# Xiaoming-Zhao/PointNav-VO

Hardware: AMD Instinct MI355X
Metric: RGB-D frame-pair VO inferences/s @341x192 (higher is better)
Workload: dtype f32

## Files before the change

### pointnav-vo_amd/csrc/pnvo_api.hip

```cpp
#include <hip/hip_runtime.h>

#include <cmath>
#include <cstdio>
#include <cstdlib>
#include <cstring>
#include <functional>
#include <atomic>
#include <condition_variable>
#include <map>
#include <mutex>
#include <string>
#include <thread>
#include <vector>

#include "pnvo_model.h"

using namespace pnvo;

thread_local std::string g_err;

int pnvo_fail(pnvo_handle h, int code, const std::string &msg) {
  if (h) h->err = msg;
  g_err = msg;
  return code;
}

long long pnvo_device_bytes_live(void) { return g_device_bytes_live.load(); }

namespace {

inline int fail(pnvo_handle h, int code, const std::string &msg) { return pnvo_fail(h, code, msg); }


Layer make_layer(const std::string &name, const std::string &gn, int cin, int cout, int k, int stride, int pad,
                 int hin, int win, int groups) {
  Layer l;
  l.name = name;
  l.gn = gn;
  l.cin = cin;
  l.cinp = rup(cin, 8);
  l.cout = cout;
  l.coutp = rup(cout, 32);
  l.k = l.kw = k;
  l.stride = stride;
  l.pad = pad;
  l.hin = hin;
  l.win = win;
  l.hout = (hin + 2 * pad - k) / stride + 1;
  l.wout = (win + 2 * pad - k) / stride + 1;
  l.groups = groups;
  return l;
}

void build_plan(pnvo_model_s *m) {
  const pnvo_config &c = m->cfg;
  m->C = c.n_rgb + c.n_depth + c.n_dd + c.n_tdv;
  m->CP = rup(m->C, 8);
  m->CPL = rup(m->C, 16);
  m->Hs = halve(c.height);
  m->Ws = halve(c.width);
  m->Hp = halve(m->Hs);
  m->Wp = halve(m->Ws);
  {
    const int n[4] = {c.n_rgb, c.n_depth, c.n_dd, c.n_tdv};
    int prev_off[4], half = 0;
    for (int t = 0; t < 4; ++t) {
      prev_off[t] = half;
      half += n[t] / 2;
    }
    m->stem_ref_of_new.clear();
    m->stem_tensor_of_new.clear();
    m->stem_ch_of_new.clear();
    for (int t = 0; t < 4; ++t)
      for (int ch = 0; ch < n[t]; ++ch) {
        const int hn = n[t] / 2;
        m->stem_ref_of_new.push_back(ch < hn ? prev_off[t] + ch : half + prev_off[t] + (ch - hn));
        m->stem_tensor_of_new.push_back(t);
        m->stem_ch_of_new.push_back(ch);
      }
    while ((int)m->stem_ref_of_new.size() < m->CP) {
      m->stem_ref_of_new.push_back(-1);
      m->stem_tensor_of_new.push_back(-1);
      m->stem_ch_of_new.push_back(0);
    }
  }
  const int g = c.baseplanes / 2;
  const std::string bb = "visual_encoder.backbone.";
  m->convs.clear();
  m->convs.push_back(make_layer(bb + "conv1.0", bb + "conv1.1", m->C, c.baseplanes, 7, 2, 3, c.height, c.width, g));
  int h = m->Hp, w = m->Wp, cin = c.baseplanes;
  const bool bott = c.backbone_depth == 50 || c.backbone_depth == 101;
  const int nblk[4] = {bott ? 3 : 2, bott ? 4 : 2, bott ? (c.backbone_depth == 101 ? 23 : 6) : 2, bott ? 3 : 2};
  const bool resnext = bott && c.resnext != 0, se = bott && c.se != 0;
  const int expansion = resnext ? 2 : 4, cardinality = resnext ? c.baseplanes / 2 : 1;
  m->bottleneck = bott;
  m->grouped_se = resnext || se;
  m->blocks.clear();
  auto push = [&](Layer l) {
    l.block = (int)m->blocks.size();
    m->convs.push_back(std::move(l));
    return (int)m->convs.size() - 1;
  };
  for (int st = 1; st <= 4; ++st) {
    const int planes = (resnext ? 2 * c.baseplanes : c.baseplanes) << (st - 1), cout = bott ? planes * expansion : planes;
    for (int bi = 0; bi < nblk[st - 1]; ++bi) {
      Block b;
      b.stage = st;
      b.index = bi;
      b.tap = "layer" + std::to_string(st) + "." + std::to_string(bi);
      const std::string p = bb + b.tap + ".";
      const int stride = (st > 1 && bi == 0) ? 2 : 1;
      if (bott) {
        Layer b2 = make_layer(p + "convs.3", p + "convs.4", planes, planes, 3, stride, 1, h, w, g);
        b.nconv = 3;
        b.conv[0] = push(make_layer(p + "convs.0", p + "convs.1", cin, planes, 1, 1, 0, h, w, g));
        if (bi == 0) b2.cgroups = cardinality;
        const int h2 = b2.hout, w2 = b2.wout;
        b.conv[1] = push(std::move(b2));
        if (se) b.se_r = cout / 16;
        b.conv[2] = push(make_layer(p + "convs.6", p + "convs.7", planes, cout, 1, 1, 0, h2, w2, g));
      } else {
        Layer c1 = make_layer(p + "convs.0", p + "convs.1", cin, planes, 3, stride, 1, h, w, g);
        b.nconv = 2;
        const int h1 = c1.hout, w1 = c1.wout;
        b.conv[0] = push(std::move(c1));
        b.conv[1] = push(make_layer(p + "convs.3", p + "convs.4", planes, planes, 3, 1, 1, h1, w1, g));
      }
      if (stride != 1 || cin != cout) b.ds = push(make_layer(p + "downsample.0", p + "downsample.1", cin, cout, 1, stride, 0, h, w, g));
      m->blocks.push_back(std::move(b));
      h = m->last(m->blocks.back()).hout;
      w = m->last(m->blocks.back()).wout;
      cin = cout;
    }
  }
  m->fh = h;
  m->fw = w;
  m->comp_c = (int)std::lround((double)c.flat_size / (double)(h * w));
  {
    const double q = (double)c.flat_size / (double)(h * w);
    const double fl = std::floor(q);
    if (q - fl == 0.5) m->comp_c = ((long)fl % 2 == 0) ? (int)fl : (int)fl + 1;
  }
  m->comp_cp = rup(m->comp_c, 32);
  m->comp = (int)m->convs.size();
  m->convs.push_back(make_layer("visual_encoder.compression.0", "visual_encoder.compression.1", cin, m->comp_c, 3, 1, 1,
                                h, w, 1));
  m->fc = make_layer(c.act_embed ? "hidden_generator.1" : "visual_fc.2", "", m->comp_c, c.hidden, 1, 1, 0, h, w, 1);
  m->fc.cinp = m->comp_cp;
  m->fc.k = h;
  m->fc.kw = w;
  m->fc.hout = m->fc.wout = 1;
  m->head = make_layer("output_head.1", "", c.hidden, c.out_dim, 1, 1, 0, 1, 1, 1);
}

struct Toc {
  std::map<std::string, const pnvo_tensor_desc *> by_name;
  const float *blob;
  size_t n;
};

const float *find_tensor(pnvo_handle h, const Toc &t, const std::string &name, std::vector<int64_t> shape, int *rc) {
  auto it = t.by_name.find(name);
  if (it == t.by_name.end()) {
    *rc = fail(h, PNVO_ERR_WEIGHTS, "state_dict is missing tensor '" + name + "'");
    return nullptr;
  }
  const pnvo_tensor_desc *d = it->second;
// ... 684 lines not shown
static int stem_launch_mx(pnvo_handle m, int B, const StemRequest &r, const StemPlan &p, GnGroup &sgg) {
  const Layer &stem = m->convs[0];
  StemMXArgs a;
  std::memset(&a, 0, sizeof(a));
  pnvo_stem_mx_input(m, B, r.src, r.raw, a);
  a.wpk = p.pieces == 2 ? m->mx_wpk2 : m->mx_wpk3;
  a.oscale = m->mx_oscale;
  a.oscale_ptr = m->mx_wpk2_dev ? m->mx_scale2_dev + 1 : nullptr;
  a.bad_input = m->dd_flag_dev;
  const int ntn = stem.cout / 32;
  for (int g = 0; g < ntn; ++g) {
    a.y[g] = r.y;
    a.stats[g] = m->stats;
    a.y_coff[g] = 32 * g;
  }
  a.y_cstride = stem.coutp;
  a.stats_cstride = stem.coutp;
  a.pool = r.pool_keys;
  a.pool_gamma = stem.gamma;
  a.Hp = m->Hp;
  a.Wp = m->Wp;
  if (r.grp != nullptr) {
    if (p.pieces != 2 || r.pool_keys == nullptr) return fail(m, PNVO_ERR_STATE, "grouped forward needs the float16-piece stem with pooled keys");
    a.grp_end0 = sgg.end0 = r.grp->end[0];
    if (r.grp->n > 2) a.grp_end1 = sgg.end1 = r.grp->end[1];
    for (int k = 1; k < r.grp->n; ++k) {
      pnvo_handle hk = r.grp->h[k];
      if (hk->mx_wpk2 == nullptr || hk->mx_wpk2_dev) return fail(m, PNVO_ERR_STATE, "grouped forward: a model has no host-packed float16 stem operand");
      a.wpk_g[k - 1] = hk->mx_wpk2;
      a.oscale_g[k - 1] = hk->mx_oscale;
      a.pool_gamma_g[k - 1] = sgg.gamma[k - 1] = hk->convs[0].gamma;
      sgg.beta[k - 1] = hk->convs[0].beta;
    }
  }
  a.dbg = m->opt.stem_dbg >= 16 ? m->opt.stem_dbg - 16 : 0;
  if (m->opt.stem_dbg == 9 || m->opt.stem_dbg >= 16) {
    if (!m->mx_prof) {
      HIPCHK(m, m->mx_prof.alloc(256));
      HIPCHK(m, hipMemset(m->mx_prof, 0, 2048));
    }
    a.prof = m->mx_prof;
  }
  if (p.standin) return pnvo_stem_standin(m, B, r, p.slots, nullptr);
  Timed t = stem_timed(m, B, r, false);
  return pnvo_launch_stem_mx(m, a, p.pieces, ntn, false, r.grp, r.s);
}

static int stem_launch_dd(pnvo_handle m, int B, const StemRequest &r, const StemPlan &p) {
  const pnvo_config &c = m->cfg;
  if (p.standin) return pnvo_stem_standin(m, B, r, p.slots, nullptr);
  const int nsrc[4] = {c.n_rgb, c.n_depth, c.n_dd, c.n_tdv};
  StemDDArgs a;
  std::memset(&a, 0, sizeof(a));
  for (int j = 0; j < 3; ++j)
    for (int q = 0; q < 2; ++q) {
      const int d = 4 * j + 2 * q;
      const int tn = m->dd_dense_tensor[d];
      a.pieces[j][0][q].base = tn >= 0 ? r.src[tn] : nullptr;
      a.pieces[j][0][q].nch = tn >= 0 ? nsrc[tn] : 0;
      a.pieces[j][0][q].choff = tn >= 0 ? m->dd_dense_ch[d] : 0;
    }
  a.sc = m->dd_sc;
  a.sh = m->dd_sh;
  a.wpk = m->dd_wpk;
  a.table = m->dd_table;
  a.dd = r.src[2];
  a.zero_page = m->zero_page;
  a.bad_onehot = m->dd_flag_dev;
  a.y = r.y;
  a.stats = m->stats;
  a.B = B;
  a.H = c.height;
  a.W = c.width;
  a.Ho = m->Hs;
  a.Wo = m->Ws;
  a.bins = m->dd_bins;
  a.slots = p.slots;
  a.dbg = m->opt.stem_dbg;
  if (a.dbg == 9) {
    if (!m->dd_prof) {
      HIPCHK(m, m->dd_prof.alloc(8));
      HIPCHK(m, hipMemset(m->dd_prof, 0, 64));
    }
    a.prof = m->dd_prof;
  }
  Timed t = stem_timed(m, B, r, false);
  HIPCHK(m, launch_stem_dd(a, r.s));
  return PNVO_OK;
}

int pnvo_run_stem(pnvo_handle m, int B, const StemRequest &r) {
  const Layer &stem = m->convs[0];
  const StemPlan p = pnvo_stem_plan(m, r.train_fwd, r.raw);
  int rc = PNVO_OK;
  if (r.pool_keys != nullptr && !p.pools()) return fail(m, PNVO_ERR_STATE, "pooled stem output asked of a stem kernel without it");
  GnGroup sgg{0x7fffffff, 0x7fffffff, {nullptr, nullptr}, {nullptr, nullptr}};
  switch (p.kernel) {
    case StemPlan::MX: rc = stem_launch_mx(m, B, r, p, sgg); break;
    case StemPlan::DD: rc = stem_launch_dd(m, B, r, p); break;
    case StemPlan::LDS: {
      StemArgs a;
      stem_lds_args(m, B, r, p.slots, a);
      a.dbg = m->opt.stem_dbg;
      a.lds_pad = m->opt.stem_dbg_pad;
      Timed t = stem_timed(m, B, r, false);
      HIPCHK(m, launch_stem_lds(a, stem.coutp, r.s));
      break;
    }
    case StemPlan::GENERIC:
      return pnvo_run_conv(m, stem, B, {.in_scale = m->stem_sc, .in_shift = m->stem_sh, .y = r.y, .y_cstride = stem.coutp, .ss = r.ss,
                                        .mu = r.mu, .rstd = r.rstd, .src = r.src, .grp = r.grp, .s = r.s});
  }
  if (rc != PNVO_OK) return rc;
  if (p.kernel != StemPlan::LDS) {
    if (p.repairs && (rc = pnvo_stem_standin(m, B, r, p.slots, m->dd_flag_dev)) != PNVO_OK) return rc;
    if ((rc = pnvo_mark_stem(m, r.s, p)) != PNVO_OK) return rc;
  }
  if (r.slots_out != nullptr) *r.slots_out = p.slots;
  if (!r.skip_finalize) {
    Timed t(m, r.s, "gn_finalize", 0.0, 0.0);
    HIPCHK(m, launch_gn_finalize(m->stats, B, p.slots, stem.coutp, stem.cout, stem.groups, (long)m->Hs * m->Ws, 1, stem.gamma, stem.beta,
                                 1e-5f, r.ss[0], r.ss[1], r.s, p.slots, r.mu, r.rstd, r.grp ? &sgg : nullptr));
  }
  return PNVO_OK;
}

int pnvo_ensure_workspace(pnvo_handle m, int B) { return ensure_workspace(m, B); }

namespace {
struct OptChoice {
  const char *word;
  int value;
};
struct OptDef {
  const char *key, *env;
  int PnvoOptions::*field;
  bool numeric;
  OptChoice choices[7];
};
const OptDef kOptions[] = {
    {"stem", "PNVO_STEM", &PnvoOptions::stem, false, {{"auto", 0}, {"mx", 1}, {"dd", 2}, {"dense", 3}, {nullptr, 0}}},
    {"conv", "PNVO_CONV", &PnvoOptions::conv, false, {{"auto", 0}, {"x3", 1}, {"fp32", 2}, {"generic", 3}, {nullptr, 0}}},
    {"pieces", "PNVO_PIECES", &PnvoOptions::pieces, false, {{"2", 2}, {"3", 3}, {nullptr, 0}}},
    {"stem_form", "PNVO_STEM_FORM", &PnvoOptions::stem_form, false, {{"auto", 0}, {"tiles", 2}, {"resident", 3}, {"fast", 4}, {nullptr, 0}}},
    {"train_pieces", "PNVO_TRAIN_PIECES", &PnvoOptions::train_pieces, false, {{"2", 2}, {"3", 3}, {nullptr, 0}}},
    {"x3_persist", "PNVO_X3_PERSIST", &PnvoOptions::x3_persist, false, {{"on", 1}, {"off", 0}, {nullptr, 0}}},
    {"x3_rows", "PNVO_X3_ROWS", &PnvoOptions::x3_rows, false, {{"on", 1}, {"off", 0}, {nullptr, 0}}},
    {"x3_strip", "PNVO_X3_STRIP", &PnvoOptions::x3_strip, false, {{"on", 1}, {"off", 0}, {nullptr, 0}}},
    {"x3_fine", "PNVO_X3_FINE", &PnvoOptions::x3_fine, false, {{"on", 1}, {"off", 0}, {nullptr, 0}}},
    {"x3_w8", "PNVO_X3_W8", &PnvoOptions::x3_w8, false, {{"on", 1}, {"off", 0}, {nullptr, 0}}},
    {"x3_m16", "PNVO_X3_M16", &PnvoOptions::x3_m16, false, {{"on", 1}, {"off", 0}, {nullptr, 0}}},
    {"x3_ksplit", "PNVO_X3_KSPLIT", &PnvoOptions::x3_ksplit, false, {{"on", 1}, {"off", 0}, {nullptr, 0}}},
    {"fc_rows", "PNVO_FC_ROWS", &PnvoOptions::fc_rows, true, {{nullptr, 0}}},
    {"head_fuse", "PNVO_HEAD_FUSE", &PnvoOptions::head_fuse, false, {{"on", 1}, {"off", 0}, {nullptr, 0}}},
    {"ds_fuse", "PNVO_DS_FUSE", &PnvoOptions::ds_fuse, false, {{"on", 1}, {"off", 0}, {nullptr, 0}}},
    {"gn_fuse", "PNVO_GN_FUSE", &PnvoOptions::gn_fuse, false, {{"on", 1}, {"off", 0}, {nullptr, 0}}},
    {"x3_s2", nullptr, &PnvoOptions::x3_s2, false, {{"on", 1}, {"off", 0}, {nullptr, 0}}},
    {"tail", "PNVO_TAIL", &PnvoOptions::tail, false, {{"fused", 1}, {"separate", 0}, {nullptr, 0}}},
    {"pool", "PNVO_POOL", &PnvoOptions::pool, false, {{"fused", 1}, {"separate", 0}, {nullptr, 0}}},
    {"graph", "PNVO_GRAPH", &PnvoOptions::graph, true, {{nullptr, 0}}},
    {"stem_dbg", nullptr, &PnvoOptions::stem_dbg, true, {{nullptr, 0}}},
    {"stem_dbg_pad", nullptr, &PnvoOptions::stem_dbg_pad, true, {{nullptr, 0}}},
    {"wgrad_stem", "PNVO_WGRAD_STEM", &PnvoOptions::wgrad_stem, false, {{"mx", 0}, {"fp32", 1}, {nullptr, 0}}},
    {"wgrad3", "PNVO_WGRAD3", &PnvoOptions::wgrad3, false, {{"x3", 1}, {"fp32", 0}, {nullptr, 0}}},
    {"pool_bwd", "PNVO_POOL_BWD", &PnvoOptions::pool_bwd, false, {{"fused", 1}, {"separate", 0}, {nullptr, 0}}},
    {"dgrad", "PNVO_DGRAD", &PnvoOptions::dgrad, false, {{"phase", 1}, {"masked", 0}, {nullptr, 0}}},
    {"bf16_fuse", nullptr, &PnvoOptions::bf16_fuse, false, {{"on", 1}, {"off", 0}, {nullptr, 0}}},
    {"input_fallback", "PNVO_INPUT_FALLBACK", &PnvoOptions::input_fallback, false, {{"on", 1}, {"off", 0}, {nullptr, 0}}},
    {"small_net", "PNVO_SMALL_NET", &PnvoOptions::small_net, false, {{"on", 1}, {"off", 0}, {nullptr, 0}}},
    {"small_max", "PNVO_SMALL_MAX", &PnvoOptions::small_max, true, {{nullptr, 0}}},
    {"small_coop", "PNVO_SMALL_COOP", &PnvoOptions::small_coop, true, {{nullptr, 0}}},
    {"small_prof", "PNVO_SMALL_PROF", &PnvoOptions::small_prof, true, {{nullptr, 0}}},
};

const OptDef *find_option(const char *key) {
  for (const OptDef &d : kOptions)
    if (std::strcmp(d.key, key) == 0) return &d;
  return nullptr;
}

bool parse_option(const OptDef &d, const char *word, int *out) {
  if (d.numeric) {
    char *end = nullptr;
    const long v = std::strtol(word, &end, 10);
    if (end == word || *end != 0) return false;
    *out = (int)v;
    return true;
  }
  for (const OptChoice *c = d.choices; c->word != nullptr; ++c)
    if (std::strcmp(c->word, word) == 0) {
      *out = c->value;
      return true;
    }
  return false;
}

void env_defaults(pnvo_model_s *m) {
  for (const OptDef &d : kOptions) {
    const char *e = d.env ? std::getenv(d.env) : nullptr;
    int v;
    if (e && parse_option(d, e, &v)) m->opt.*(d.field) = v;
  }
  if (std::getenv("PNVO_X3_S2_OFF")) m->opt.x3_s2 = 0;
  if (std::getenv("PNVO_BF16_NOFUSE")) m->opt.bf16_fuse = 0;
  if (const char *e = std::getenv("PNVO_STEM_DBG")) std::sscanf(e, "%d,%d", &m->opt.stem_dbg, &m->opt.stem_dbg_pad);
}
}


int pnvo_input_fallback(pnvo_handle m, hipStream_t s, bool *rerun) {
  *rerun = false;
  if (!m->stem_ev_pending) return PNVO_OK;
  m->stem_ev_pending = false;
  HIPCHK(m, hipEventSynchronize(m->stem_ev));
  if (!m->dd_flag || *(volatile int *)m->dd_flag == 0) return PNVO_OK;
  *(volatile int *)m->dd_flag = 0;
  HIPCHK(m, hipMemsetAsync(m->dd_flag_dev, 0, sizeof(int), s));
  m->dense_sticky = true;
  m->fallback_count += 1;
  pnvo_drop_graphs(m);
  m->note = "note: observation values outside the fused stems' contract (fractional rgb or depth codes that are not one-hot) — "
           "the forward was re-run on the dense fp32 stem and this handle stays on it";
  *rerun = true;
  return PNVO_OK;
}

namespace {
int forward_dispatch(pnvo_handle m, int B, const FwdRequest &r);
int forward_body(pnvo_handle m, int B, const FwdRequest &r);
}


extern "C" {

#include "src_hash.h"
const char *pnvo_version(void) { return "pnvo 0.3 (gfx950: fp32 + f16/bf16 MFMA) src:" PNVO_SRC_HASH; }

const char *pnvo_last_error(pnvo_handle h) { return h ? h->err.c_str() : g_err.c_str(); }

const char *pnvo_last_note(pnvo_handle h) {
  if (h && h->loaded && h->opt.input_fallback && pnvo_stem_plan(h, false, {}).lds_serves) (void)pnvo_check_inputs(h);
  return h ? h->note.c_str() : "";
}

int pnvo_create(const pnvo_config *cfg, int device, pnvo_handle *out) {
  if (!cfg || !out) return fail(nullptr, PNVO_ERR_ARG, "null argument");
  const int C = cfg->n_rgb + cfg->n_depth + cfg->n_dd + cfg->n_tdv;
  if (C <= 0) return fail(nullptr, PNVO_ERR_ARG, "visual odometry must not be blind (no input modality)");
  if (C > 64 || (cfg->n_rgb % 2) || (cfg->n_depth % 2) || (cfg->n_dd % 2) || (cfg->n_tdv % 2))
    return fail(nullptr, PNVO_ERR_ARG, "unsupported input channel configuration");
  if (cfg->width < 32 || cfg->height < 32) return fail(nullptr, PNVO_ERR_ARG, "observation_size must be >= 32x32");
  if (cfg->baseplanes < 32 || cfg->baseplanes % 32 || cfg->hidden % 8 || cfg->hidden <= 0 || cfg->out_dim <= 0)
    return fail(nullptr, PNVO_ERR_ARG, "unsupported baseplanes / hidden_size / output_dim");
  if ((cfg->resnext != 0 && cfg->resnext != 1) || (cfg->se != 0 && cfg->se != 1) ||
      ((cfg->resnext || cfg->se) && cfg->backbone_depth != 50 && cfg->backbone_depth != 101))
    return fail(nullptr, PNVO_ERR_ARG, "unsupported backbone: resnext / se are 0 or 1 and need backbone_depth 50 or 101");
  hipError_t e = hipSetDevice(device);
  if (e != hipSuccess) return fail(nullptr, PNVO_ERR_HIP, std::string("hipSetDevice: ") + hipGetErrorString(e));
  hipDeviceProp_t prop;
  e = hipGetDeviceProperties(&prop, device);
  if (e != hipSuccess) return fail(nullptr, PNVO_ERR_HIP, std::string("hipGetDeviceProperties: ") + hipGetErrorString(e));
  if (std::string(prop.gcnArchName).rfind("gfx950", 0) != 0)
    return fail(nullptr, PNVO_ERR_ARG, std::string("libpnvo is built for gfx950 only, device is ") + prop.gcnArchName);
  pnvo_model_s *m = new pnvo_model_s();
  static std::atomic<unsigned long long> next_uid{1};
  m->uid = next_uid.fetch_add(1);
  m->cfg = *cfg;
  m->device = device;
  m->num_cus = prop.multiProcessorCount;
  if (m->cfg.flat_size <= 0) m->cfg.flat_size = 2048;
  if (m->cfg.n_acts <= 0) m->cfg.n_acts = 4;
  env_defaults(m);
  build_plan(m);
  *out = m;
  return PNVO_OK;
}

int pnvo_load_weights(pnvo_handle h, const float *blob, size_t n_floats, const pnvo_tensor_desc *toc, int ntoc) {
  if (!h || !blob || !toc) return fail(h, PNVO_ERR_ARG, "null argument");
  HIPCHK(h, hipSetDevice(h->device));
  pnvo_drop_graphs(h);
  Toc t;
  t.blob = blob;
  t.n = n_floats;
  for (int k = 0; k < ntoc; ++k) t.by_name[toc[k].name] = &toc[k];
  int rc = PNVO_OK;
  const pnvo_config &c = h->cfg;
  h->mean.assign(h->C, 0.f);
  h->stdev.assign(h->C, 1.f);
  if (c.normalize) {
    const std::string pre = "visual_encoder.running_mean_and_var.";
    const float *mu = find_tensor(h, t, pre + "_mean", {1, h->C, 1, 1}, &rc);
    if (!mu) return rc;
    const float *var = find_tensor(h, t, pre + "_var", {1, h->C, 1, 1}, &rc);
    if (!var) return rc;
    for (int k = 0; k < h->C; ++k) {
      h->mean[k] = mu[k];
      h->stdev[k] = std::sqrt(std::fmax(var[k], 1e-2f));
    }
  }
  for (Layer &l : h->convs)
    if ((rc = load_conv(h, t, l, true)) != PNVO_OK) return rc;
  for (Block &b : h->blocks) {
    if (b.se_r == 0) continue;
    const std::string pre = "visual_encoder.backbone." + b.tap + ".se.excite.";
    const int C = h->last(b).cout, R = b.se_r;
    if (!se_gate_supported(C, R)) return fail(h, PNVO_ERR_ARG, "SE branch of " + b.tap + ": unsupported width " + std::to_string(C));
// ... 496 lines not shown
      if (b.se_r > 0) {
        if (b3.cout != b3.coutp) return fail(m, PNVO_ERR_STATE, "SE block " + b.tap + " on a channel-padded map");
        Timed t(m, s, "se_gate:" + b.tap, 2.0 * B * (2.0 * b.se_r + (double)Pb) * b3.cout, 4.0 * B * Pb * b3.cout);
        HIPCHK(m, launch_se_gate({.x = m->rawB, .scale = m->ssA[0], .shift = m->ssA[1], .w1 = b.se_w1, .b1 = b.se_b1, .w2 = b.se_w2,
                                  .b2 = b.se_b2, .out_scale = m->ssE[0], .out_shift = m->ssE[1], .B = B, .P = (int)Pb, .C = b3.cout,
                                  .R = b.se_r}, s));
        ss3 = m->ssE;
      }
      if (ds) {
        const Layer &cd = m->convs[b.ds];
        if ((rc = pnvo_run_conv(m, cd, B, {.x = cur, .y = m->rawD, .y_cstride = cd.coutp, .ss = m->ssD, .grp = grp, .s = s})) != PNVO_OK)
          return rc;
        Timed t(m, s, "residual", 0.0, 12.0 * B * Pb * b3.coutp);
        HIPCHK(m, launch_residual(m->rawB, ss3[0], ss3[1], m->rawD, m->ssD[0], m->ssD[1], B, Pb, b3.coutp, nxt, s));
      } else {
        Timed t(m, s, "residual", 0.0, 12.0 * B * Pb * b3.coutp);
        HIPCHK(m, launch_residual(m->rawB, ss3[0], ss3[1], cur, nullptr, nullptr, B, Pb, b3.coutp, nxt, s));
      }
      std::swap(cur, nxt);
      if ((rc = maybe_tap(m, b.tap.c_str(), cur, (size_t)B * Pb * b3.coutp, s)) != PNVO_OK) return rc;
      continue;
    }
    const Layer &c1 = m->convs[b.conv[0]];
    const Layer &c2 = m->convs[b.conv[1]];
    const bool ds_ride = ds && !have_keys && pnvo_conv_takes_ds(m, c1, m->convs[b.ds], B);
    const DsRide ride{ds_ride ? &m->convs[b.ds] : nullptr, m->rawD, m->ssD, nullptr, nullptr};
    if (have_keys) {
      BlockTail ktail{nullptr, nullptr, nullptr, cur};
      if ((rc = pnvo_run_conv(m, c1, B, {.x = nxt, .in_scale = m->ssA[0], .in_shift = m->ssA[1], .y = m->rawA, .y_cstride = c1.coutp,
                                         .ss = m->ssA, .tail = &ktail, .grp = grp, .s = s})) != PNVO_OK)
        return rc;
      have_keys = false;
    } else if (have_tail) {
      if (ds_ride) tail.out = nullptr;
      if ((rc = pnvo_run_conv(m, c1, B, {.x = m->rawB, .in_scale = m->ssB[0], .in_shift = m->ssB[1], .y = m->rawA, .y_cstride = c1.coutp,
                                         .ss = m->ssA, .tail = &tail, .ride = ds_ride ? &ride : nullptr, .grp = grp, .s = s})) != PNVO_OK)
        return rc;
      std::swap(cur, nxt);
      have_tail = false;
    } else if ((rc = pnvo_run_conv(m, c1, B, {.x = cur, .y = m->rawA, .y_cstride = c1.coutp, .ss = m->ssA, .ride = ds_ride ? &ride : nullptr,
                                              .grp = grp, .s = s})) != PNVO_OK) {
      return rc;
    }
    const long P = (long)c2.hout * c2.wout;
    const bool c2_small_generic = !layer_on_lds(m, c2, nullptr) && !pnvo_conv_on_x3(m, c2, B) && (size_t)B * P * c2.cinp * 4 <= ((size_t)48 << 20);
    if (c2_small_generic) {
      float *napp = ds_ride ? nxt : m->rawD;
      {
        Timed t(m, s, "gn_relu_apply", 0.0, 8.0 * B * P * c2.cinp);
        HIPCHK(m, launch_apply_ss_relu(m->rawA, m->ssA[0], m->ssA[1], B, P, c2.cinp, napp, s));
      }
      if ((rc = pnvo_run_conv(m, c2, B, {.x = napp, .y = m->rawB, .y_cstride = c2.coutp, .ss = m->ssB, .grp = grp, .s = s})) != PNVO_OK)
        return rc;
    } else if ((rc = pnvo_run_conv(m, c2, B, {.x = m->rawA, .in_scale = m->ssA[0], .in_shift = m->ssA[1], .y = m->rawB, .y_cstride = c2.coutp,
                                              .ss = m->ssB, .grp = grp, .s = s})) != PNVO_OK) {
      return rc;
    }
    if (ds) {
      const Layer &cd = m->convs[b.ds];
      if (!ds_ride &&
          (rc = pnvo_run_conv(m, cd, B, {.x = cur, .y = m->rawD, .y_cstride = cd.coutp, .ss = m->ssD, .grp = grp, .s = s})) != PNVO_OK)
        return rc;
    }
    if (pnvo_conv_takes_tail(m, m->convs[m->next_conv_after(bk)], B)) {
      tail.res = ds ? m->rawD : cur;
      tail.res_scale = ds ? m->ssD[0] : nullptr;
      tail.res_shift = ds ? m->ssD[1] : nullptr;
      tail.out = nxt;
      have_tail = true;
      continue;
    }
    {
      Timed t(m, s, "residual", 0.0, 12.0 * B * P * c2.coutp);
      HIPCHK(m, launch_residual(m->rawB, m->ssB[0], m->ssB[1], ds ? m->rawD : cur, ds ? m->ssD[0] : nullptr, ds ? m->ssD[1] : nullptr, B,
                                P, c2.coutp, nxt, s));
    }
    std::swap(cur, nxt);
    if ((rc = maybe_tap(m, b.tap.c_str(), cur, (size_t)B * P * c2.coutp, s)) != PNVO_OK) return rc;
  }

  const Layer &comp = m->convs[m->comp];
  if (have_tail) {
    tail.out = nullptr;
    if ((rc = pnvo_run_conv(m, comp, B, {.x = m->rawB, .in_scale = m->ssB[0], .in_shift = m->ssB[1], .y = m->comp_raw, .y_cstride = comp.coutp,
                                         .ss = m->ssC, .tail = &tail, .grp = grp, .s = s})) != PNVO_OK)
      return rc;
    have_tail = false;
  } else if ((rc = pnvo_run_conv(m, comp, B, {.x = cur, .y = m->comp_raw, .y_cstride = comp.coutp, .ss = m->ssC, .grp = grp, .s = s})) != PNVO_OK) {
    return rc;
  }
  if (m->tap_dst != nullptr && m->tap_name == "compression") {
    HIPCHK(m, launch_apply_ss_relu(m->comp_raw, m->ssC[0], m->ssC[1], B, (long)m->fh * m->fw, m->comp_cp, m->tapbuf, s));
    if ((rc = maybe_tap(m, "compression", m->tapbuf, (size_t)B * m->fh * m->fw * m->comp_cp, s)) != PNVO_OK) return rc;
  }
  if (r.stop_after_compression) return PNVO_OK;
  if (grp != nullptr) {
    bool rows_ok = !c.act_embed;
    FwdRequest rk = r;
    rk.actions = nullptr;
    for (int k = 0; k < grp->n; ++k) rows_ok = rows_ok && fc_rows_usable(grp->h[k], B, rk);
    if (rows_ok) return run_fc_rows(m, grp->h, grp->end, grp->n, B, m->comp_raw, m->ssC[0], m->ssC[1], rk);
    int start = 0;
    for (int k = 0; k < grp->n; ++k) {
      const int Bk = grp->end[k] - start;
      pnvo_handle hk = grp->h[k];
      if (k > 0 && (rc = ensure_workspace(hk, Bk)) != PNVO_OK) return fail(m, rc, std::string("grouped forward: ") + pnvo_last_error(hk));
      const size_t crow = (size_t)m->fh * m->fw * m->comp_cp;
      rk.out = r.out + (size_t)start * c.out_dim;
      rc = run_fc_head(hk, Bk, m->comp_raw + start * crow, m->ssC[0] + (size_t)start * m->comp_cp, m->ssC[1] + (size_t)start * m->comp_cp, rk);
      if (rc != PNVO_OK) return k > 0 ? fail(m, rc, std::string("grouped forward: ") + pnvo_last_error(hk)) : rc;
      start = grp->end[k];
    }
    return PNVO_OK;
  }
  return run_fc_head(m, B, m->comp_raw, m->ssC[0], m->ssC[1], r);
}

bool fc_rows_usable(pnvo_handle m, int B, const FwdRequest &r) {
  const long kp = (long)m->fh * m->fw * m->comp_cp;
  return m->opt.fc_rows >= B && B >= 1 && m->fc_rows_w != nullptr && m->train == nullptr && m->precision == 0 && m->opt.conv == 0 &&
         m->comp_cp > 0 && 256 % m->comp_cp == 0 && kp % 4 == 0 && kp / 4 <= 64L * FC_ROWS_MAXV && m->cfg.hidden % 4 == 0 &&
         (r.features_only || m->head_w_plain != nullptr);
}

int run_fc_rows(pnvo_handle m, pnvo_handle const *grp, const int *end, int ng, int B, const float *comp_raw, const float *sc, const float *sh,
                const FwdRequest &r) {
  const pnvo_config &c = m->cfg;
  FcRowsArgs a;
  std::memset(&a, 0, sizeof(a));
  a.x = comp_raw;
  a.sc = sc;
  a.sh = sh;
  a.hid = r.features_only ? r.out : m->hid;
  a.out = r.out;
  a.actions = c.act_embed ? r.actions : nullptr;
  a.B = B;
  a.Kp = m->fh * m->fw * m->comp_cp;
  a.cp = m->comp_cp;
  a.hidden = c.hidden;
  a.out_dim = c.out_dim;
  a.ngroups = ng;
  for (int k = 0; k < ng; ++k) {
    a.end[k] = end[k];
    a.w[k] = grp[k]->fc_rows_w;
    a.bias[k] = grp[k]->fc_bias;
    a.head_w[k] = grp[k]->head_w_plain;
    a.head_b[k] = grp[k]->head_bias;
  }
  Timed t(m, r.s, "conv:" + m->fc.name, 2.0 * B * (double)a.Kp * c.hidden, 4.0 * ng * (double)a.Kp * c.hidden);
  HIPCHK(m, launch_fc_rows(a, !r.features_only, r.s));
  return PNVO_OK;
}

int run_fc_head(pnvo_handle m, int B, const float *comp_raw, const float *sc, const float *sh, const FwdRequest &r) {
  const pnvo_config &c = m->cfg;
  float *out = r.out;
  hipStream_t s = r.s;
  int rc = PNVO_OK;
  if (fc_rows_usable(m, B, r)) {
    pnvo_handle one[1] = {m};
    const int end[1] = {B};
    if ((rc = run_fc_rows(m, one, end, 1, B, comp_raw, sc, sh, r)) != PNVO_OK) return rc;
    return r.features_only ? PNVO_OK : maybe_tap(m, "hidden", m->hid, (size_t)B * c.hidden, s);
  }
  bool head_rode = false;
  const float *head_w = m->train != nullptr ? pnvo_train_weight_ptr(m, "output_head.1.weight") : m->head_w_plain;
  float *head_out = (m->opt.head_fuse && !r.features_only && c.out_dim <= 4 && head_w != nullptr) ? out : nullptr;
  if ((rc = pnvo_run_conv(m, m->fc, B, {.x = comp_raw, .in_scale = sc, .in_shift = sh, .y = m->hid, .y_cstride = c.hidden, .bias = m->fc_bias,
                                        .bias_row = c.act_embed ? r.actions : nullptr, .relu_out = 1, .head_w = head_w, .head_out = head_out,
                                        .head_rode = &head_rode, .s = s})) != PNVO_OK)
    return rc;
  if ((rc = maybe_tap(m, "hidden", m->hid, (size_t)B * c.hidden, s)) != PNVO_OK) return rc;
  if (head_rode) return PNVO_OK;
  if (r.features_only) {
    HIPCHK(m, hipMemcpyAsync(out, m->hid, (size_t)B * c.hidden * sizeof(float), hipMemcpyDeviceToDevice, s));
    return PNVO_OK;
  }
  return pnvo_run_conv(m, m->head, B, {.x = m->hid, .y = out, .y_cstride = c.out_dim, .bias = m->head_bias, .s = s});
}
}

namespace {
bool raw_direct(pnvo_handle m, const float *depth_frames) {
  const StemPlan sp = pnvo_stem_plan(m, false, {});
  if (depth_frames == nullptr || !sp.raw_stager() || m->tap_dst != nullptr) return false;
  if (m->precision == 1) return true;
  return sp.h2_from_host;
}

int raw_materialise(pnvo_handle m, const uint8_t *rgb_frames, const float *depth_frames, int B, int32_t *err_flag, hipStream_t s) {
  const pnvo_config &c = m->cfg;
  if (B > m->rawws_cap) {
    for (DevBuf<float> &q : m->rawws) q.reset();
    const size_t px = (size_t)B * c.height * c.width;
    if (c.n_rgb) HIPCHK(m, m->rawws[0].alloc(px * 6));
    HIPCHK(m, m->rawws[1].alloc(px * 2));
    if (c.n_dd) HIPCHK(m, m->rawws[2].alloc(px * (size_t)c.n_dd));
    m->rawws_cap = B;
  }
  HIPCHK(m, launch_frame_pairs(c.n_rgb ? rgb_frames : nullptr, depth_frames, B, c.height, c.width, c.n_dd / 2, m->rawws[0], m->rawws[1],
                               m->rawws[2], err_flag, s));
  return PNVO_OK;
}
}

int pnvo_forward_raw(pnvo_handle m, const uint8_t *rgb_frames, const float *depth_frames, const float *tdv, const int64_t *actions, int B,
                     float *out, int32_t *err_flag, void *stream) {
  if (!m) return fail(m, PNVO_ERR_ARG, "null handle");
  if (!m->loaded) return fail(m, PNVO_ERR_STATE, "pnvo_forward_raw before pnvo_load_weights");
  if (B <= 0 || !out) return fail(m, PNVO_ERR_ARG, "bad batch / null output");
  const pnvo_config &c = m->cfg;
  if ((c.n_rgb > 0) != (rgb_frames != nullptr) || ((c.n_depth > 0 || c.n_dd > 0) && depth_frames == nullptr) ||
      (c.n_tdv > 0) != (tdv != nullptr))
    return fail(m, PNVO_ERR_ARG, "sensor frames do not match the model's observation_space");
  if (c.act_embed && !actions) return fail(m, PNVO_ERR_ARG, "act_embed model needs actions");
  if (int rc0 = pnvo_check_inputs(m)) return rc0;
  HIPCHK(m, hipSetDevice(m->device));
  hipStream_t s = (hipStream_t)stream;
  if (!raw_direct(m, depth_frames)) {
    int rc = raw_materialise(m, rgb_frames, depth_frames, B, err_flag, s);
    if (rc != PNVO_OK) return rc;
    return pnvo_forward(m, c.n_rgb ? m->rawws[0] : nullptr, c.n_depth ? m->rawws[1] : nullptr, c.n_dd ? m->rawws[2] : nullptr, tdv,
                        actions, B, out, stream);
  }
  const FwdRequest r{.src = {nullptr, nullptr, nullptr, tdv}, .raw = {rgb_frames, depth_frames, err_flag}, .actions = actions, .out = out, .s = s};
  if (m->precision == 1) {
    pnvo_handle hs[1] = {m};
    float *outs[1] = {out};
    return pnvo_forward_bf16(hs, 1, B, r, outs);
  }
  int rc = ensure_workspace(m, B);
  if (rc == PNVO_OK) rc = forward_dispatch(m, B, r);
  m->stem_ev_pending = false;
  return rc;
}

int pnvo_grouped_supported(const pnvo_handle *hs, int n) {
  if (!hs || n < 1 || n > 3 || !hs[0]) return fail(nullptr, PNVO_ERR_ARG, "bad handle list");
  pnvo_handle m = hs[0];
  const pnvo_config &c = m->cfg;
  for (int k = 0; k < n; ++k) {
    pnvo_handle h = hs[k];
    if (!h) return fail(m, PNVO_ERR_ARG, "grouped forward: null handle");
    for (int j = 0; j < k; ++j)
      if (hs[j] == h) return fail(m, PNVO_ERR_ARG, "grouped forward: a handle appears twice");
    if (!h->loaded) return fail(m, PNVO_ERR_STATE, "grouped forward before pnvo_load_weights");
    if (std::memcmp(&h->cfg, &c, sizeof(pnvo_config)) != 0 || h->device != m->device)
      return fail(m, PNVO_ERR_ARG, "the models of a grouped forward must share architecture and device");
    const StemPlan sp = pnvo_stem_plan(h, false, {});
    if (h->precision != 0 || h->train != nullptr || h->bottleneck || c.act_embed || !sp.raw_stager() || !sp.h2_from_host ||
        h->tap_dst != nullptr || !h->opt.pool || !h->opt.tail || h->opt.conv > 1)
      return fail(m, PNVO_ERR_STATE, "grouped forward needs float32 inference handles on the default float16-piece kernels (no training step, "
                                     "no tap, no act-embed, options pieces=2 / stem=auto / conv=auto / pool / tail at their defaults)");
    for (size_t li = 1; li < h->convs.size(); ++li)
      if (h->convs[li].groups > 0 && !x3_two_pieces(h, h->convs[li]))
        return fail(m, PNVO_ERR_STATE, "grouped forward: layer " + h->convs[li].name + " of a model is range-guarded off the float16-piece form");
  }
  return PNVO_OK;
}

int pnvo_forward_grouped_raw(const pnvo_handle *handles, const int32_t *counts, int n_models, const uint8_t *rgb_frames,
                             const float *depth_frames, const float *tdv, int B, float *out, int32_t *err_flag, void *stream) {
  if (!handles || !counts || n_models < 1 || n_models > 3 || !handles[0]) return fail(nullptr, PNVO_ERR_ARG, "bad handle list");
  pnvo_handle hs[3] = {nullptr, nullptr, nullptr};
  int cnt[3] = {0, 0, 0}, ng = 0, total = 0;
  for (int k = 0; k < n_models; ++k) {
    if (counts[k] < 0 || (counts[k] > 0 && !handles[k])) return fail(handles[0], PNVO_ERR_ARG, "bad pair count / null handle");
    total += counts[k];
    if (counts[k] > 0) {
      hs[ng] = handles[k];
      cnt[ng++] = counts[k];
    }
  }
  pnvo_handle m = hs[0];
  if (ng == 0 || total != B || B <= 0 || !out) return fail(handles[0], PNVO_ERR_ARG, "pair counts do not add up to the batch / null output");
  if (ng == 1) return pnvo_forward_raw(m, rgb_frames, depth_frames, tdv, nullptr, B, out, err_flag, stream);
  const pnvo_config &c = m->cfg;
  if (int rcs = pnvo_grouped_supported(hs, ng)) return rcs;
  for (int k = 0; k < ng; ++k)
    if (int rc0 = pnvo_check_inputs(hs[k])) return rc0;
  if ((c.n_rgb > 0) != (rgb_frames != nullptr) || ((c.n_depth > 0 || c.n_dd > 0) && depth_frames == nullptr) || (c.n_tdv > 0) != (tdv != nullptr))
    return fail(m, PNVO_ERR_ARG, "sensor frames do not match the models' observation_space");
  if (!raw_direct(m, depth_frames)) return fail(m, PNVO_ERR_STATE, "grouped forward needs the sensor-frame stager of the float16-piece stem");
  HIPCHK(m, hipSetDevice(m->device));
  hipStream_t s = (hipStream_t)stream;
  int rc = ensure_workspace(m, B);
  if (rc != PNVO_OK) return rc;
  const PnvoOptions saved = m->opt;
  m->opt.conv = 1;
  m->opt.x3_rows = 0;
  m->opt.x3_persist = 0;
  GroupedFwd grp{ng, {hs[0], hs[1], hs[2]}, {0, 0, 0}};
  for (int k = 0, acc = 0; k < ng; ++k) grp.end[k] = acc += cnt[k];
  rc = forward_body(m, B, {.src = {nullptr, nullptr, nullptr, tdv}, .raw = {rgb_frames, depth_frames, err_flag}, .out = out, .grp = &grp, .s = s});
  m->stem_ev_pending = false;
  m->opt = saved;
  return rc;
}

int pnvo_forward_dual_raw(pnvo_handle ha, pnvo_handle hb, const uint8_t *rgb_frames, const float *depth_frames, const float *tdv, int B,
                          float *out_a, float *out_b, int32_t *err_flag, void *stream) {
  if (!ha || !hb) return fail(ha, PNVO_ERR_ARG, "null handle");
  if (!ha->loaded || !hb->loaded) return fail(ha, PNVO_ERR_STATE, "pnvo_forward_dual_raw before pnvo_load_weights");
  if (B <= 0 || !out_a || !out_b) return fail(ha, PNVO_ERR_ARG, "bad batch / null output");
  if (ha->precision != 1 || hb->precision != 1)
    return fail(ha, PNVO_ERR_STATE, "pnvo_forward_dual_raw runs the bfloat16 path: call pnvo_set_precision(h, 1) on both models");
  if (std::memcmp(&ha->cfg, &hb->cfg, sizeof(pnvo_config)) != 0 || ha->device != hb->device)
    return fail(ha, PNVO_ERR_ARG, "the two models of a dual forward must share architecture and device");
  const pnvo_config &c = ha->cfg;
  if (c.act_embed) return fail(ha, PNVO_ERR_ARG, "pnvo_forward_dual_raw covers the separate-action models");
  if ((c.n_rgb > 0) != (rgb_frames != nullptr) || ((c.n_depth > 0 || c.n_dd > 0) && depth_frames == nullptr) ||
      (c.n_tdv > 0) != (tdv != nullptr))
    return fail(ha, PNVO_ERR_ARG, "sensor frames do not match the model's observation_space");
  HIPCHK(ha, hipSetDevice(ha->device));
  hipStream_t s = (hipStream_t)stream;
  if (!raw_direct(ha, depth_frames)) {
    int rc = raw_materialise(ha, rgb_frames, depth_frames, B, err_flag, s);
// ... 402 lines not shown
```

### pointnav-vo_amd/csrc/pnvo_model.h

```cpp
#pragma once
#include <hip/hip_runtime.h>

#include <map>
#include <functional>
#include <string>
#include <vector>

#include "../../include/pnvo.h"
#include "pnvo_internal.h"
#include "dev_buf.h"

using pnvo::DevBuf;
using pnvo::DevPair;

static inline int rup(int x, int m) { return (x + m - 1) / m * m; }
static inline int halve(int x) { return (x - 1) / 2 + 1; }

struct Layer {
  std::string name, gn;
  int cin = 0, cinp = 0, cout = 0, coutp = 0, k = 1, kw = 1, stride = 1, pad = 0;
  int hin = 0, win = 0, hout = 0, wout = 0, groups = 1;
  DevBuf<float> wpk, gamma, beta;
  std::vector<float> host_w;
  DevBuf<unsigned short> wpk_x3;
  unsigned long long x3_gen = 0;
  DevBuf<unsigned short> wpk_x2;
  unsigned long long x2_gen = 0;
  float x2_oscale = 1.f;
  float in_bound = 3.0e38f;
  int block = -1;
  int cgroups = 1;
  DevBuf<float> wpk_grp;
};

struct Block {
  int stage = 0, index = 0;
  int nconv = 0;
  int conv[3] = {-1, -1, -1};
  int ds = -1;
  std::string tap;
  int se_r = 0;
  DevBuf<float> se_w1, se_b1, se_w2, se_b2;
};

struct PnvoOptions {
  int stem = 0;
  int conv = 0;
  int stem_form = 0;
  int pieces = 2;
  int train_pieces = 2;
  int x3_rows = 1;
  int x3_persist = 1;
  int x3_strip = 1;
  int x3_fine = 1;
  int x3_m16 = 1;
  int x3_w8 = 1;
  int x3_ksplit = 1;
  int fc_rows = 48;
  int head_fuse = 1;
  int ds_fuse = 1;
  int gn_fuse = 1;
  int x3_s2 = 1;
  int tail = 1;
  int pool = 1;
  int graph = 0;
  int stem_dbg = 0, stem_dbg_pad = 0;
  int wgrad_stem = 0;
  int wgrad3 = 1;
  int pool_bwd = 1;
  int dgrad = 1;
  int bf16_fuse = 1;
  int input_fallback = 1;
  int small_net = 1;
  int small_max = 3;
  int small_prof = 0;
  int small_coop = 1;
};

struct TimingRec {
  hipEvent_t a, b;
  int entry;
};

struct pnvo_model_s {
  pnvo_config cfg;
  int device = 0;
  std::string err;
  std::string note;
  bool loaded = false;

  int C = 0, CP = 0;
  int Hs = 0, Ws = 0, Hp = 0, Wp = 0, fh = 0, fw = 0, comp_c = 0, comp_cp = 0;
  std::vector<Layer> convs;
  std::vector<Block> blocks;
  int comp = -1;
  const Layer &last(const Block &b) const { return convs[b.conv[b.nconv - 1]]; }
  int next_conv_after(size_t k) const { return k + 1 < blocks.size() ? blocks[k + 1].conv[0] : comp; }
  Layer fc, head;
  DevBuf<float> fc_bias, head_bias;
  DevBuf<float> fc_rows_w;
  DevBuf<float> head_w_plain;
  std::vector<float> mean, stdev;
  std::vector<int> stem_ref_of_new;
  std::vector<int> stem_tensor_of_new, stem_ch_of_new;
  DevBuf<float> stem_sc, stem_sh, zero_page;
  DevBuf<float> kpart;
  DevBuf<float> stem_wpk16;
  int CPL = 0;
  bool dd_ok = false;
  int dd_bins = 0;
  std::vector<int> dd_dense_tensor, dd_dense_ch;
  DevBuf<float> dd_wpk, dd_table, dd_sc, dd_sh;
  DevBuf<int> dd_flag;
  DevBuf<int> dd_flag_dev;
  DevBuf<unsigned long long> dd_prof;

  bool mx_ok = false;
  DevBuf<unsigned short> mx_wpk3;
  DevBuf<unsigned short> mx_wpk2;
  float mx_oscale = 1.f;
  DevBuf<float> mx_scale2_dev;
  bool mx_wpk2_dev = false;
  std::vector<float> mx_wk, mx_wk_swapped;
  int mx_xslot[4] = {-1, -1, -1, -1};
  std::vector<int> mx_slot_ref, mx_slot_new;
  DevBuf<float> mx_pages;
  DevBuf<unsigned long long> mx_prof;
  bool mx_prof_rs = false;
  int num_cus = 256;
  bool train_mx = false;
  PnvoOptions opt;
  bool dense_sticky = false;
  int fallback_count = 0;
  DevBuf<float> stats_ds;
  hipEvent_t stem_ev = nullptr;
  bool stem_ev_pending = false;
  DevBuf<float> rawws[3];
  int rawws_cap = 0;
  int precision = 0;
  unsigned long long load_gen = 0;
  unsigned long long weights_gen_at_load = 0;
  unsigned long long uid = 0;
  unsigned long long weights_gen = 0;
  void *bf = nullptr;

  int cap = 0;
  DevBuf<float> xin, stem_raw, bufY[2];
  DevBuf<float> rawA, rawB, rawD, rawC, comp_raw, hid, stats;
  bool bottleneck = false;
  bool grouped_se = false;
  DevPair<float> ssA, ssB, ssD, ssC;
  DevPair<float> ssE;
  DevBuf<float> tapbuf;

  std::string tap_name;
  float *tap_dst = nullptr;
  size_t tap_cap = 0;

  void *train = nullptr;
  void *small = nullptr;

  struct GraphEntry {
    const void *key[8];
    int B;
    hipGraph_t graph;
    hipGraphExec_t exec;
    unsigned long long stamp;
  };
  std::vector<GraphEntry> graphs;
  std::vector<GraphEntry> seen;
  DevBuf<float> out_ws;
  hipStream_t cap_stream = nullptr;
  int graph_mode = -1;
  unsigned long long graph_clock = 0;

  int timing = 0;
  std::vector<pnvo_kernel_time> tentries;
  std::map<std::string, int> tindex;
  std::vector<TimingRec> trecs;
  std::vector<hipEvent_t> evpool;
};


struct BlockTail {
  const float *res, *res_scale, *res_shift;
  float *out;
};

struct DsRide {
  const Layer *cd;
  float *y;
  float *const *ss;
  float *mu, *rstd;
};

struct GroupedFwd {
  int n;
  pnvo_model_s *h[3];
  int end[3];
};

struct ConvRequest {
  const float *x = nullptr;
  const float *in_scale = nullptr, *in_shift = nullptr;
  float *y = nullptr;
  int y_cstride = 0;
  float *const *ss = nullptr;
  float *mu = nullptr, *rstd = nullptr;
  const float *bias = nullptr;
  const int64_t *bias_row = nullptr;
  int relu_out = 0;
// ... 98 lines not shown
```

Baseline: 118,100.

## Add MFMA split-K FC GEMM kernel with fused GroupNorm-ReLU input for large batches

Adds a dedicated fp32 MFMA (32x32x2) GEMM kernel for the final fully connected layer when the batch exceeds the fc_rows threshold. It applies the per-channel scale/shift and ReLU on the fly to the compressed features, caching these tables in shared memory, and splits K into four slices. The slices are reduced by the existing ksplit reduce-with-head kernel. This replaces the generic conv path for the FC at large batch, trading an extra partial-sum buffer and a reduce pass for better matrix-core use.

Result: no change. 118,200 (median of 2 runs) (+0.1%).

```diff
diff --git a/pointnav-vo_amd/csrc/fc_gemm.h b/pointnav-vo_amd/csrc/fc_gemm.h
--- /dev/null
+++ b/pointnav-vo_amd/csrc/fc_gemm.h
@@ -0,0 +1,20 @@
+#pragma once
+#include <hip/hip_runtime.h>
+
+namespace pnvo {
+
+constexpr int FC_GEMM_MAX_CP = 128;
+constexpr int FC_GEMM_SLICES = 4;
+
+struct FcGemmArgs {
+  const float *x;
+  const float *sc, *sh;
+  const float *w;
+  float *part;
+  int B, Kp, cp, hidden;
+};
+
+bool fc_gemm_supported(int B, int Kp, int cp, int hidden);
+hipError_t launch_fc_gemm(const FcGemmArgs &a, hipStream_t s);
+
+}
diff --git a/pointnav-vo_amd/csrc/fc_gemm.hip b/pointnav-vo_amd/csrc/fc_gemm.hip
--- /dev/null
+++ b/pointnav-vo_amd/csrc/fc_gemm.hip
@@ -0,0 +1,102 @@
+#include "fc_gemm.h"
+
+namespace pnvo {
+
+typedef float f32x4 __attribute__((ext_vector_type(4)));
+typedef float f32x16 __attribute__((ext_vector_type(16)));
+
+constexpr int FC_GEMM_U = 8;
+
+template <bool TAB>
+__global__ __launch_bounds__(256) void fc_gemm_kernel(const FcGemmArgs p) {
+  constexpr int U = FC_GEMM_U;
+  extern __shared__ float tab[];
+  __shared__ float red[4 * 1024];
+  const int tid = (int)threadIdx.x, lane = tid & 63, wave = tid >> 6;
+  const int i = lane & 31, h = lane >> 5;
+  const int n0 = (int)blockIdx.x * 32, b0 = (int)blockIdx.y * 32, z = (int)blockIdx.z;
+  const int cp = p.cp, ts = cp + 4;
+  if constexpr (TAB) {
+    for (int e = tid; e < 32 * cp; e += 256) {
+      const int r = e / cp, ch = e - r * cp;
+      const long bb = min(b0 + r, p.B - 1);
+      tab[r * ts + ch] = p.sc[bb * cp + ch];
+      tab[32 * ts + r * ts + ch] = p.sh[bb * cp + ch];
+    }
+    __syncthreads();
+  }
+  const long brow = min(b0 + i, p.B - 1);
+  const float *xr = p.x + brow * p.Kp + 4 * h;
+  const float *wr = p.w + (long)(n0 + i) * p.Kp + 4 * h;
+  const float *scl = tab + i * ts, *shl = tab + 32 * ts + i * ts;
+  const float *scg = p.sc + brow * cp, *shg = p.sh + brow * cp;
+  const int S = p.Kp >> 3, q = z * 4 + wave;
+  const int s0 = (int)((long)q * S / (4 * FC_GEMM_SLICES)), s1 = (int)((long)(q + 1) * S / (4 * FC_GEMM_SLICES));
+  int c = (8 * s0 + 4 * h) % cp;
+
+  f32x16 acc;
+#pragma unroll
+  for (int r = 0; r < 16; ++r) acc[r] = 0.f;
+
+  auto load = [&](int s, f32x4(&a)[U], f32x4(&b)[U]) {
+#pragma unroll
+    for (int u = 0; u < U; ++u) {
+      const int su = min(s + u, s1 - 1);
+      a[u] = *reinterpret_cast<const f32x4 *>(xr + 8 * su);
+      b[u] = *reinterpret_cast<const f32x4 *>(wr + 8 * su);
+    }
+  };
+  auto mac = [&](int s, const f32x4(&a)[U], const f32x4(&b)[U]) {
+#pragma unroll
+    for (int u = 0; u < U; ++u) {
+      if (s + u < s1) {
+        const f32x4 scv = *reinterpret_cast<const f32x4 *>((TAB ? scl : scg) + c), shv = *reinterpret_cast<const f32x4 *>((TAB ? shl : shg) + c);
+#pragma unroll
+        for (int t = 0; t < 4; ++t)
+          acc = __builtin_amdgcn_mfma_f32_32x32x2f32(fmaxf(__builtin_fmaf(a[u][t], scv[t], shv[t]), 0.f), b[u][t], acc, 0, 0, 0);
+        c += 8;
+        if (c >= cp) c -= cp;
+      }
+    }
+  };
+  if (s0 < s1) {
+    f32x4 a0[U], b0v[U], a1[U], b1v[U];
+    load(s0, a0, b0v);
+    for (int s = s0; s < s1; s += 2 * U) {
+      if (s + U < s1) load(s + U, a1, b1v);
+      mac(s, a0, b0v);
+      if (s + U < s1) {
+        if (s + 2 * U < s1) load(s + 2 * U, a0, b0v);
+        mac(s + U, a1, b1v);
+      }
+    }
+  }
+
+#pragma unroll
+  for (int r = 0; r < 16; ++r) red[wave * 1024 + r * 64 + lane] = acc[r];
+  __syncthreads();
+  float *part = p.part + (long)z * p.B * p.hidden;
+#pragma unroll
+  for (int j = 0; j < 4; ++j) {
+    const int e = tid + 256 * j, r = e >> 6, l = e & 63;
+    const float v = ((red[e] + red[1024 + e]) + red[2048 + e]) + red[3072 + e];
+    const int b = b0 + (r & 3) + 8 * (r >> 2) + 4 * (l >> 5);
+    if (b < p.B) part[(long)b * p.hidden + n0 + (l & 31)] = v;
+  }
+}
+
+bool fc_gemm_supported(int B, int Kp, int cp, int hidden) {
+  return B >= 1 && hidden >= 32 && hidden % 32 == 0 && Kp >= 8 && Kp % 8 == 0 && cp >= 8 && cp % 4 == 0 && Kp % cp == 0;
+}
+
+hipError_t launch_fc_gemm(const FcGemmArgs &a, hipStream_t s) {
+  if (!fc_gemm_supported(a.B, a.Kp, a.cp, a.hidden)) return hipErrorInvalidValue;
+  const dim3 grid((unsigned)(a.hidden / 32), (unsigned)((a.B + 31) / 32), (unsigned)FC_GEMM_SLICES);
+  if (a.cp <= FC_GEMM_MAX_CP)
+    hipLaunchKernelGGL(fc_gemm_kernel<true>, grid, dim3(256), (size_t)2 * 32 * (a.cp + 4) * sizeof(float), s, a);
+  else
+    hipLaunchKernelGGL(fc_gemm_kernel<false>, grid, dim3(256), 0, s, a);
+  return hipGetLastError();
+}
+
+}
diff --git a/pointnav-vo_amd/csrc/pnvo_api.hip b/pointnav-vo_amd/csrc/pnvo_api.hip
--- a/pointnav-vo_amd/csrc/pnvo_api.hip
+++ b/pointnav-vo_amd/csrc/pnvo_api.hip
@@ -13,6 +13,7 @@
 #include <thread>
 #include <vector>
 
+#include "fc_gemm.h"
 #include "pnvo_model.h"
 
 using namespace pnvo;
@@ -1003,7 +1004,8 @@
     {"x3_m16", "PNVO_X3_M16", &PnvoOptions::x3_m16, false, {{"on", 1}, {"off", 0}, {nullptr, 0}}},
     {"x3_ksplit", "PNVO_X3_KSPLIT", &PnvoOptions::x3_ksplit, false, {{"on", 1}, {"off", 0}, {nullptr, 0}}},
     {"fc_rows", "PNVO_FC_ROWS", &PnvoOptions::fc_rows, true, {{nullptr, 0}}},
-    {"head_fuse", "PNVO_HEAD_FUSE", &PnvoOptions::head_fuse, false, {{"on", 1}, {"off", 0}, {nullptr, 0}}},
+    {"fc_gemm", "PNVO_FC_GEMM", &PnvoOptions::fc_gemm, false, {{"on", 1}, {"off", 0}, {nullptr, 0}}},
+    {"head_fuse", "PNVO_HEAD_FUSE",&PnvoOptions::head_fuse, false, {{"on", 1}, {"off", 0}, {nullptr, 0}}},
     {"ds_fuse", "PNVO_DS_FUSE", &PnvoOptions::ds_fuse, false, {{"on", 1}, {"off", 0}, {nullptr, 0}}},
     {"gn_fuse", "PNVO_GN_FUSE", &PnvoOptions::gn_fuse, false, {{"on", 1}, {"off", 0}, {nullptr, 0}}},
     {"x3_s2", nullptr, &PnvoOptions::x3_s2, false, {{"on", 1}, {"off", 0}, {nullptr, 0}}},
@@ -1806,6 +1808,41 @@
   return PNVO_OK;
 }
 
+bool fc_gemm_usable(pnvo_handle m, int B, const FwdRequest &r) {
+  const pnvo_config &c = m->cfg;
+  return m->opt.fc_gemm && B > m->opt.fc_rows && m->fc_rows_w != nullptr && m->train == nullptr && m->precision == 0 && m->opt.conv == 0 &&
+         r.grp == nullptr && !r.features_only && m->opt.head_fuse && c.out_dim <= 4 && m->head_w_plain != nullptr &&
+         fc_gemm_supported(B, m->fh * m->fw * m->comp_cp, m->comp_cp, c.hidden);
+}
+
+int run_fc_gemm(pnvo_handle m, int B, const float *comp_raw, const float *sc, const float *sh, const FwdRequest &r) {
+  const pnvo_config &c = m->cfg;
+  const size_t need = (size_t)FC_GEMM_SLICES * B * c.hidden;
+  if (need > m->kpart.size()) {
+    pnvo_drop_graphs(m);
+    HIPCHK(m, m->kpart.alloc(need));
+  }
+  const FcGemmArgs g{.x = comp_raw, .sc = sc, .sh = sh, .w = m->fc_rows_w, .part = m->kpart, .B = B, .Kp = m->fh * m->fw * m->comp_cp,
+                     .cp = m->comp_cp, .hidden = c.hidden};
+  ConvArgs a;
+  std::memset(&a, 0, sizeof(a));
+  a.B = B;
+  a.Ho = a.Wo = 1;
+  a.COUT = a.y_cstride = c.hidden;
+  a.y = m->hid;
+  a.bias = m->fc_bias;
+  a.bias_row = c.act_embed ? r.actions : nullptr;
+  a.relu_out = 1;
+  a.kpart = m->kpart;
+  a.ksplit = FC_GEMM_SLICES;
+  {
+    Timed t(m, r.s, "conv:" + m->fc.name, conv_flops(m->fc, B), conv_bytes(m->fc, B));
+    HIPCHK(m, launch_fc_gemm(g, r.s));
+    HIPCHK(m, launch_ksplit_reduce_head(a, m->head_w_plain, m->head_bias, c.out_dim, r.out, r.s));
+  }
+  return maybe_tap(m, "hidden", m->hid, (size_t)B * c.hidden, r.s);
+}
+
 int run_fc_head(pnvo_handle m, int B, const float *comp_raw, const float *sc, const float *sh, const FwdRequest &r) {
   const pnvo_config &c = m->cfg;
   float *out = r.out;
@@ -1817,6 +1854,7 @@
     if ((rc = run_fc_rows(m, one, end, 1, B, comp_raw, sc, sh, r)) != PNVO_OK) return rc;
     return r.features_only ? PNVO_OK : maybe_tap(m, "hidden", m->hid, (size_t)B * c.hidden, s);
   }
+  if (fc_gemm_usable(m, B, r)) return run_fc_gemm(m, B, comp_raw, sc, sh, r);
   bool head_rode = false;
   const float *head_w = m->train != nullptr ? pnvo_train_weight_ptr(m, "output_head.1.weight") : m->head_w_plain;
   float *head_out = (m->opt.head_fuse && !r.features_only && c.out_dim <= 4 && head_w != nullptr) ? out : nullptr;
diff --git a/pointnav-vo_amd/csrc/pnvo_model.h b/pointnav-vo_amd/csrc/pnvo_model.h
--- a/pointnav-vo_amd/csrc/pnvo_model.h
+++ b/pointnav-vo_amd/csrc/pnvo_model.h
@@ -57,6 +57,7 @@
   int x3_w8 = 1;
   int x3_ksplit = 1;
   int fc_rows = 48;
+  int fc_gemm = 1;
   int head_fuse = 1;
   int ds_fuse = 1;
   int gn_fuse = 1;
```
